# maybeLx/MVSFormerPlusPlus

Measured on NVIDIA H100. Metric: depth-maps/sec (hot path: FMT + 4-stage cascade), higher is better.
Workload: dtype f32

## Files before the change

### mvsformerplusplus_b200/csrc/attention_fa.cuh

```cuda
#pragma once

namespace fa {
using namespace gmma;
constexpr int NCONS = 256, THREADS = NCONS + 32, NKV = 3;
constexpr uint32_t TILE = 4096;
constexpr uint32_t LBO_QK = 2048, LBO_V = 640;
constexpr uint32_t V_TILE = 16 * LBO_V;
constexpr uint32_t OFF_Q = 0, OFF_K = 2 * TILE, OFF_V = OFF_K + NKV * 2 * TILE, OFF_BAR = OFF_V + NKV * V_TILE;
constexpr uint32_t SMEM = OFF_BAR + 8 + 32 * NKV;
}

__global__ void qkv_tile_kernel(const float* __restrict__ qkv, __half* __restrict__ tiled, int N, int ntiles, float qscale) {
  const int i = blockIdx.x * blockDim.x + threadIdx.x;
  const int total = ntiles * 128 * 3 * 4 * 2;
  if (i >= total) return;
  const int oct = i & 1, h = (i >> 1) & 3, which = (i >> 3) % 3, tok = i / 24;
  const size_t plane = (size_t)4 * ntiles * 2048;
  const int tile = tok >> 7, r = tok & 127;
  float v[8];
  if (tok < N) {
    const float4 a = ldg4(qkv + (size_t)tok * 192 + which * 64 + h * 16 + oct * 8);
    const float4 b = ldg4(qkv + (size_t)tok * 192 + which * 64 + h * 16 + oct * 8 + 4);
    v[0] = a.x; v[1] = a.y; v[2] = a.z; v[3] = a.w; v[4] = b.x; v[5] = b.y; v[6] = b.z; v[7] = b.w;
    if (which == 0) {
#pragma unroll
      for (int e = 0; e < 8; ++e) v[e] *= qscale;
    }
  } else {
#pragma unroll
    for (int e = 0; e < 8; ++e) v[e] = 0.f;
  }
  if (which < 2) {
    __half* ph = tiled + (size_t)(which * 2) * plane + ((size_t)h * ntiles + tile) * 2048;
    __half* pl = ph + plane;
    split_store8(ph + oct * 1024 + r * 8, pl + oct * 1024 + r * 8, v);
  } else {
    __half* pv = tiled + (size_t)4 * plane + ((size_t)h * ntiles + tile) * 5120;
    const int kc = r >> 3, e = r & 7;
#pragma unroll
    for (int d = 0; d < 8; ++d) {
      __half hi, lo;
      split_f16(v[d], hi, lo);
      pv[kc * 320 + (oct * 8 + d) * 8 + e] = lo;
      pv[kc * 320 + (16 + oct * 8 + d) * 8 + e] = hi;
    }
    if (oct == 0) {
      pv[kc * 320 + 32 * 8 + e] = __float2half_rn(1.0f);
    } else {
#pragma unroll
      for (int z = 33; z < 40; ++z) pv[kc * 320 + z * 8 + e] = __float2half_rn(0.f);
    }
  }
}

namespace fa {
using namespace gmma;
__device__ __forceinline__ void issue_scores(float (&S)[64], uint64_t q_hi, uint64_t q_lo, uint32_t kt) {
  const uint64_t k_hi = make_desc(kt, LBO_QK, 128), k_lo = make_desc(kt + TILE, LBO_QK, 128);
  mma_ss<128>(S, q_lo, k_hi, 0u);
  mma_ss<128>(S, q_hi, k_lo, 1u);
  mma_ss<128>(S, q_hi, k_hi, 1u);
  wg_commit();
}
template <bool PLO>
__device__ __forceinline__ void issue_pv(float (&O)[20], const uint32_t (&ph)[8][4], const uint32_t (&pl)[8][4], uint32_t vt) {
#pragma unroll
  for (int i = 0; i < 8; ++i) {
    mma_rs_n40(O, ph[i], make_desc(vt + 2 * i * LBO_V, LBO_V, 128), i > 0 ? 1u : 0u);
    if (PLO) mma_rs_n24(O + 8, pl[i], make_desc(vt + 2 * i * LBO_V + 256, LBO_V, 128), 1u);
  }
  wg_commit();
}
__device__ __forceinline__ void softmax_tile(float (&S)[64], float (&m)[2], float (&corr)[2], int j, int N, int q) {
  if (j * 128 + 128 > N) {
#pragma unroll
    for (int i = 0; i < 64; ++i)
      if (j * 128 + 8 * (i >> 2) + 2 * q + (i & 1) >= N) S[i] = -1e30f;
  }
  float mb[2];
#pragma unroll
  for (int h = 0; h < 2; ++h) {
    float pmax = -1e30f;
#pragma unroll
    for (int b = 0; b < 16; ++b) pmax = fmaxf(pmax, fmaxf(S[4 * b + 2 * h], S[4 * b + 2 * h + 1]));
    pmax = fmaxf(pmax, __shfl_xor_sync(0xffffffffu, pmax, 1));
    pmax = fmaxf(pmax, __shfl_xor_sync(0xffffffffu, pmax, 2));
    const float mx = fmaxf(m[h], pmax);
    corr[h] = ex2f(m[h] - mx);
    m[h] = mx;
    mb[h] = mx - 14.0f;
  }
#pragma unroll
  for (int i = 0; i < 64; ++i) S[i] = ex2f(S[i] - mb[(i >> 1) & 1]);
}
template <bool PLO>
__device__ __forceinline__ void pack_p(const float (&S)[64], uint32_t (&ph)[8][4], uint32_t (&pl)[8][4]) {
#pragma unroll
  for (int i = 0; i < 8; ++i)
#pragma unroll
    for (int r = 0; r < 4; ++r) {
      const float p0 = S[8 * i + 2 * r], p1 = S[8 * i + 2 * r + 1];
      const __half2 hh = __floats2half2_rn(p0, p1);
      ph[i][r] = *reinterpret_cast<const uint32_t*>(&hh);
      if (PLO) {
        const float2 hf = __half22float2(hh);
        pl[i][r] = pack_half2(p0 - hf.x, p1 - hf.y);
      }
    }
}
__device__ __forceinline__ void fold_tile(float (&o)[2][4], float (&l)[2], const float (&O)[20], const float (&corr)[2], int lane) {
#pragma unroll
  for (int h = 0; h < 2; ++h) {
#pragma unroll
    for (int b = 0; b < 2; ++b)
#pragma unroll
      for (int e = 0; e < 2; ++e) o[h][2 * b + e] = fmaf(o[h][2 * b + e], corr[h], O[4 * b + 2 * h + e] + O[4 * (b + 2) + 2 * h + e]);
    const float lt = __shfl_sync(0xffffffffu, O[16 + 2 * h], lane & ~3);
    l[h] = fmaf(l[h], corr[h], lt);
  }
}
}

template <bool PLO>
__global__ void __launch_bounds__(fa::THREADS, 1)
attention_fa_kernel(const __half* __restrict__ tiled, float* __restrict__ out, __half* __restrict__ out2, int N, int ntiles) {
  using namespace fa;
  extern __shared__ __align__(128) unsigned char smem[];
  const int tid = threadIdx.x, warp = tid >> 5, lane = tid & 31;
  const int head = blockIdx.y, qt = blockIdx.x;
  const size_t plane = (size_t)4 * ntiles * 2048;
  const __half* base = tiled + (size_t)head * ntiles * 2048;
  const uint32_t sb = smem_u32(smem);
  const uint32_t bar_q = sb + OFF_BAR, bar_kf = bar_q + 8, bar_ke = bar_kf + 8 * NKV, bar_vf = bar_ke + 8 * NKV,
                 bar_ve = bar_vf + 8 * NKV;
  if (tid == 0) {
    mbar_init(bar_q, 1);
    for (int i = 0; i < NKV; ++i) { mbar_init(bar_kf + 8 * i, 1); mbar_init(bar_ke + 8 * i, 2); mbar_init(bar_vf + 8 * i, 1); mbar_init(bar_ve + 8 * i, 2); }
    fence_barrier_init();
  }
  __syncthreads();

  if (warp == NCONS / 32) {
    if (lane == 0) {
      expect_tx(bar_q, 2 * TILE);
      bulk_load(sb + OFF_Q, base + 0 * plane + (size_t)qt * 2048, TILE, bar_q);
      bulk_load(sb + OFF_Q + TILE, base + 1 * plane + (size_t)qt * 2048, TILE, bar_q);
      for (int t = 0; t < ntiles; ++t) {
        const int s = t % NKV;
        const uint32_t par = (uint32_t)(((t / NKV) & 1) ^ 1);
        mbar_wait(bar_ke + 8 * s, par);
        expect_tx(bar_kf + 8 * s, 2 * TILE);
        bulk_load(sb + OFF_K + (2 * s) * TILE, base + 2 * plane + (size_t)t * 2048, TILE, bar_kf + 8 * s);
        bulk_load(sb + OFF_K + (2 * s + 1) * TILE, base + 3 * plane + (size_t)t * 2048, TILE, bar_kf + 8 * s);
        mbar_wait(bar_ve + 8 * s, par);
        expect_tx(bar_vf + 8 * s, V_TILE);
        bulk_load(sb + OFF_V + s * V_TILE, tiled + 4 * plane + ((size_t)head * ntiles + t) * (V_TILE / 2), V_TILE, bar_vf + 8 * s);
      }
    }
    return;
  }
  const int wg = warp >> 2, wq = warp & 3, q = lane & 3;
  const bool leader = (tid & 127) == 0;
  const uint64_t q_hi = make_desc(sb + OFF_Q + wg * 1024, LBO_QK, 128), q_lo = make_desc(sb + OFF_Q + TILE + wg * 1024, LBO_QK, 128);
  float o[2][4];
  float m[2] = {-1e30f, -1e30f}, l[2] = {0.f, 0.f};
#pragma unroll
  for (int h = 0; h < 2; ++h)
#pragma unroll
    for (int d = 0; d < 4; ++d) o[h][d] = 0.f;
  float S[64], O[20], corr[2];
  uint32_t ph[8][4], pl[8][4];
  mbar_wait(bar_q, 0u);
  mbar_wait(bar_kf, 0u);
  wg_fence();
  issue_scores(S, q_hi, q_lo, sb + OFF_K);
  wg_wait<0>();
  fence_regs<64>(S);
  if (leader) mbar_arrive(bar_ke);
  softmax_tile(S, m, corr, 0, N, q);
  pack_p<PLO>(S, ph, pl);
  if (ntiles > 1) {
    mbar_wait(bar_kf + 8, 0u);
    mbar_wait(bar_vf, 0u);
  }
  for (int j = 0; j + 1 < ntiles; ++j) {
    const int s = j % NKV, s1 = (j + 1) % NKV, s2 = (j + 2) % NKV;
    wg_fence();
    issue_scores(S, q_hi, q_lo, sb + OFF_K + (2 * s1) * TILE);
    issue_pv<PLO>(O, ph, pl, sb + OFF_V + s * V_TILE);
    wg_wait<1>();
    fence_regs<64>(S);
    if (leader) mbar_arrive(bar_ke + 8 * s1);
    float corr1[2];
    softmax_tile(S, m, corr1, j + 1, N, q);
    if (j + 2 < ntiles) mbar_wait(bar_kf + 8 * s2, (uint32_t)(((j + 2) / NKV) & 1));
    mbar_wait(bar_vf + 8 * s1, (uint32_t)(((j + 1) / NKV) & 1));
    wg_wait<0>();
    fence_regs<20>(O);
    if (leader) mbar_arrive(bar_ve + 8 * s);
    fold_tile(o, l, O, corr, lane);
    pack_p<PLO>(S, ph, pl);
    corr[0] = corr1[0];
    corr[1] = corr1[1];
  }
  {
    const int j = ntiles - 1, s = j % NKV;
    mbar_wait(bar_vf + 8 * s, (uint32_t)((j / NKV) & 1));
    wg_fence();
    issue_pv<PLO>(O, ph, pl, sb + OFF_V + s * V_TILE);
    wg_wait<0>();
    fence_regs<20>(O);
    fold_tile(o, l, O, corr, lane);
  }
#pragma unroll
  for (int h = 0; h < 2; ++h) {
    const int r = qt * 128 + 64 * wg + 16 * wq + (lane >> 2) + 8 * h;
    if (r >= N) continue;
    const float inv = __fdiv_rn(1.0f, l[h]);
#pragma unroll
    for (int b = 0; b < 2; ++b) {
      const int col = head * 16 + 8 * b + 2 * q;
      const float r0 = o[h][2 * b] * inv, r1 = o[h][2 * b + 1] * inv;
      if (out) *reinterpret_cast<float2*>(out + (size_t)r * 64 + col) = make_float2(r0, r1);
      if (out2) split_store2(out2 + (size_t)r * 128 + col, out2 + (size_t)r * 128 + 64 + col, r0, r1);
    }
  }
}
```

### mvsformerplusplus_b200/csrc/costreg_tr.cu

```cuda
#include <cuda_fp16.h>
#include <float.h>

#include "linear_tc.cuh"
#include "wgmma.cuh"

namespace mvsf {

constexpr int TR_PE = 0, TR_DOWN_W = 192, TR_DOWN_B = TR_DOWN_W + 64 * 256, TR_DOWN_LNW = TR_DOWN_B + 64,
              TR_DOWN_LNB = TR_DOWN_LNW + 64, TR_LAYER0 = TR_DOWN_LNB + 64;
constexpr int L_QKV = 0, L_PROJ_W = 192 * 64, L_PROJ_B = L_PROJ_W + 64 * 64, L_G1 = L_PROJ_B + 64, L_N1W = L_G1 + 64,
              L_N1B = L_N1W + 64, L_F1W = L_N1B + 64, L_F1B = L_F1W + 256 * 64, L_F2W = L_F1B + 256,
              L_F2B = L_F2W + 64 * 256, L_G2 = L_F2B + 64, L_N2W = L_G2 + 64, L_N2B = L_N2W + 64, TR_LAYER = L_N2B + 64;
constexpr int U_W = 0, U_B = 256 * 64, U_LNW = U_B + 256, U_LNB = U_LNW + 8, U_PW = U_LNB + 8, U_PB = U_PW + 8;

__global__ void pe3d_add_kernel(float* __restrict__ vol, const float* __restrict__ pos, const float* __restrict__ pe_w,
                                size_t nvox) {
  __shared__ float w[8 * 24];
  for (int i = threadIdx.x; i < 192; i += blockDim.x) w[i] = __ldg(pe_w + i);
  __syncthreads();
  size_t i = (size_t)blockIdx.x * blockDim.x + threadIdx.x;
  if (i >= nvox) return;
  const float div[4] = {1.0f, 0.1f, 0.01f, 0.001f};
  float pe[24];
#pragma unroll
  for (int a = 0; a < 3; ++a) {
    float p = __ldg(pos + a * nvox + i);
#pragma unroll
    for (int k = 0; k < 4; ++k) {
      float arg = __fmul_rn(__fmul_rn(p, 4.0f), div[k]);
      pe[a * 8 + 2 * k] = sinf(arg);
      pe[a * 8 + 2 * k + 1] = cosf(arg);
    }
  }
  float4* v = reinterpret_cast<float4*>(vol + i * 8);
  float4 v0 = v[0], v1 = v[1];
  float o[8] = {v0.x, v0.y, v0.z, v0.w, v1.x, v1.y, v1.z, v1.w};
#pragma unroll
  for (int c = 0; c < 8; ++c) {
    float s = 0.f;
#pragma unroll
    for (int k = 0; k < 24; ++k) s = fmaf(w[c * 24 + k], pe[k], s);
    o[c] += s;
  }
  v[0] = make_float4(o[0], o[1], o[2], o[3]);
  v[1] = make_float4(o[4], o[5], o[6], o[7]);
}

__global__ void patch_gather_kernel(const float* __restrict__ vol, __half* __restrict__ patches2, int D, int H, int W) {
  const int Hp = H / 4, Wp = W / 4;
  size_t total = (size_t)(D / 2) * Hp * Wp * 32;
  size_t i = (size_t)blockIdx.x * blockDim.x + threadIdx.x;
  if (i >= total) return;
  int vox = (int)(i & 31);
  size_t t = i >> 5;
  int wp = (int)(t % Wp), hp = (int)((t / Wp) % Hp), dp = (int)(t / ((size_t)Wp * Hp));
  int kw = vox & 3, kh = (vox >> 2) & 3, kd = vox >> 4;
  const float* src = vol + (((size_t)(dp * 2 + kd) * H + hp * 4 + kh) * W + wp * 4 + kw) * 8;
  float4 a = ldg4(src), b = ldg4(src + 4);
  float v[8] = {a.x, a.y, a.z, a.w, b.x, b.y, b.z, b.w};
  __half* row = patches2 + t * 512 + vox * 8;
  split_store8(row, row + 256, v);
}

__device__ __forceinline__ uint32_t pack_f16x2(float lo_elem, float hi_elem) {
  uint32_t r;
  asm("cvt.rn.f16x2.f32 %0, %1, %2;" : "=r"(r) : "f"(hi_elem), "f"(lo_elem));
  return r;
}
__device__ __forceinline__ float2 unpack_f16x2(uint32_t u) {
  __half2 h = *reinterpret_cast<__half2*>(&u);
  return __half22float2(h);
}
__device__ __forceinline__ void split_f16(float x, __half& hi, __half& lo) {
  hi = __float2half_rn(x);
  lo = __float2half_rn(x - __half2float(hi));
}
__device__ __forceinline__ float ex2f(float x) {
  float y;
  asm("ex2.approx.ftz.f32 %0, %1;" : "=f"(y) : "f"(x));
  return y;
}

#include "attention_fa.cuh"

__global__ void unpatch_ln_prob_kernel(const float* __restrict__ u, const float* __restrict__ tail,
                                       float* __restrict__ logits, int D, int H, int W) {
  const int Hp = H / 4, Wp = W / 4;
  size_t total = (size_t)D * H * W;
  size_t i = (size_t)blockIdx.x * blockDim.x + threadIdx.x;
  if (i >= total) return;
  int vox = (int)(i & 31);
  size_t t = i >> 5;
  int wp = (int)(t % Wp), hp = (int)((t / Wp) % Hp), dp = (int)(t / ((size_t)Wp * Hp));
  int kw = vox & 3, kh = (vox >> 2) & 3, kd = vox >> 4;
  float4 a = ldg4(u + i * 8), b = ldg4(u + i * 8 + 4);
  float x[8] = {a.x, a.y, a.z, a.w, b.x, b.y, b.z, b.w};
  float mean = 0.f;
#pragma unroll
  for (int c = 0; c < 8; ++c) mean += x[c];
  mean *= 0.125f;
  float var = 0.f;
#pragma unroll
  for (int c = 0; c < 8; ++c) { float dd = x[c] - mean; var = fmaf(dd, dd, var); }
  var *= 0.125f;
  const float sd = sqrtf(var + 1e-6f);
  float s = __ldg(tail + (U_PB - U_LNW));
#pragma unroll
  for (int c = 0; c < 8; ++c) {
    float y = __ldg(tail + c) * __fdiv_rn(x[c] - mean, sd) + __ldg(tail + 8 + c);
    s = fmaf(y, __ldg(tail + 16 + c), s);
  }
  logits[((size_t)(dp * 2 + kd) * H + hp * 4 + kh) * W + wp * 4 + kw] = s;
}


static int g_attention_plo = 0;

static int run_attention(const float* qkv, float* o, __half* o2, __half* tiled, int N, float scale_log2e, cudaStream_t s) {
  const int ntiles = cdiv(N, 128);
  qkv_tile_kernel<<<cdiv((long long)ntiles * 128 * 24, 256), 256, 0, s>>>(qkv, tiled, N, ntiles, scale_log2e);
  MVSF_LAUNCH_CHECK("qkv_tile");
  static DeviceOnce once;
  const int dev = current_device();
  if (once.need(dev)) {
    MVSF_CUDA_OK(cudaFuncSetAttribute(attention_fa_kernel<true>, cudaFuncAttributeMaxDynamicSharedMemorySize, (int)fa::SMEM));
    MVSF_CUDA_OK(cudaFuncSetAttribute(attention_fa_kernel<false>, cudaFuncAttributeMaxDynamicSharedMemorySize, (int)fa::SMEM));
    once.done(dev);
  }
  cudaEvent_t kt = ktimer_enabled() ? ktimer_begin("attention_tc", s) : nullptr;
  const dim3 grid(ntiles, 4);
  if (g_attention_plo)
    attention_fa_kernel<true><<<grid, fa::THREADS, fa::SMEM, s>>>(tiled, o, o2, N, ntiles);
  else
    attention_fa_kernel<false><<<grid, fa::THREADS, fa::SMEM, s>>>(tiled, o, o2, N, ntiles);
  if (kt) ktimer_end(kt, s);
  MVSF_LAUNCH_CHECK("attention_tc");
  return MVSF_OK;
}

}

using namespace mvsf;

extern "C" {

int mvsf_costreg_tr_workspace_bytes(int C, int D, int H, int W, size_t* bytes) {
  MVSF_REQUIRE(bytes && C == 8, "costreg_tr: base channel must be 8");
  MVSF_REQUIRE(D % 2 == 0 && H % 4 == 0 && W % 4 == 0 && D > 0 && H > 0 && W > 0,
               "costreg_tr: D %% 2, H %% 4, W %% 4 must be 0 (down_rate (2,4,4))");
  size_t N = (size_t)(D / 2) * (H / 4) * (W / 4);
  *bytes = (N * (256 + 64 + 64 + 64 + 64 + 64 + 192) + (N + 128) * 224) * sizeof(float);
  return MVSF_OK;
}

int mvsf_costreg_tr_forward(float* volume, const float* pos, const float* wts, const void* wts16, size_t n_wts,
                            float* logits, void* workspace, size_t workspace_bytes, int C, int D, int H, int W,
                            int layers, float softmax_scale, mvsf_stream_t stream) {
  MVSF_REQUIRE(volume && wts && wts16 && logits && workspace && layers >= 0, "costreg_tr: bad arguments");
  size_t need = 0;
  int rc = mvsf_costreg_tr_workspace_bytes(C, D, H, W, &need);
  if (rc) return rc;
  if (workspace_bytes < need) return fail(MVSF_ERR_WORKSPACE, "costreg_tr: workspace %zu < %zu bytes", workspace_bytes, need);
  MVSF_REQUIRE(((uintptr_t)workspace & 15) == 0 && ((uintptr_t)wts & 15) == 0 && ((uintptr_t)volume & 15) == 0 &&
                   ((uintptr_t)wts16 & 15) == 0 && (n_wts % 8) == 0,
               "costreg_tr: pointers must be 16-byte aligned");
  MVSF_REQUIRE(n_wts >= (size_t)TR_LAYER0 + (size_t)layers * TR_LAYER + U_PB + 1, "costreg_tr: weight blob too small");
  cudaStream_t s = (cudaStream_t)stream;
  const size_t nvox = (size_t)D * H * W;
  const int N = (int)((size_t)(D / 2) * (H / 4) * (W / 4));
  const __half* wh = reinterpret_cast<const __half*>(wts16);
  const __half* wl = wh + n_wts;
  float* big = (float*)workspace;
  __half* big2 = reinterpret_cast<__half*>(big);
  float* x = big + (size_t)N * 256;
  float* y = x + (size_t)N * 64;
  __half* x2 = reinterpret_cast<__half*>(y + (size_t)N * 64);
  __half* y2 = x2 + (size_t)N * 128;
  __half* o2 = y2 + (size_t)N * 128;
  float* qkv = reinterpret_cast<float*>(o2 + (size_t)N * 128);
  __half* split = reinterpret_cast<__half*>(qkv + (size_t)N * 192);

  if (pos) {
    pe3d_add_kernel<<<cdiv((long long)nvox, 256), 256, 0, s>>>(volume, pos, wts + TR_PE, nvox);
    MVSF_LAUNCH_CHECK("pe3d_add");
  }
  patch_gather_kernel<<<cdiv((long long)N * 32, 256), 256, 0, s>>>(volume, big2, D, H, W);
  MVSF_LAUNCH_CHECK("patch_gather");

  TcLinArgs a{};
  a.Ah = big2; a.Al = big2 + 256; a.lda = 512; a.Bh = wh + TR_DOWN_W; a.Bl = wl + TR_DOWN_W; a.ldb = 256;
  a.M = N; a.N = 64; a.K = 256; a.bias = wts + TR_DOWN_B; a.ln_w = wts + TR_DOWN_LNW; a.ln_b = wts + TR_DOWN_LNB; a.ln_eps = 1e-6f;
  a.C = x; a.ldc = 64; a.C2 = x2; a.ldc2 = 128;
  if ((rc = launch_linear_tc(a, LIN_LN, s))) return rc;

  const float scale_log2e = softmax_scale * 1.4426950408889634f;
  for (int l = 0; l < layers; ++l) {
    const size_t lo = (size_t)TR_LAYER0 + (size_t)l * TR_LAYER;
    const float* lw = wts + lo;
    TcLinArgs q{};
    q.Ah = x2; q.Al = x2 + 64; q.lda = 128; q.Bh = wh + lo + L_QKV; q.Bl = wl + lo + L_QKV; q.ldb = 64;
    q.M = N; q.N = 192; q.K = 64; q.C = qkv; q.ldc = 192;
    if ((rc = launch_linear_tc(q, LIN_BIAS, s))) return rc;
    if ((rc = run_attention(qkv, nullptr, o2, split, N, scale_log2e, s))) return rc;
    TcLinArgs p{};
    p.Ah = o2; p.Al = o2 + 64; p.lda = 128; p.Bh = wh + lo + L_PROJ_W; p.Bl = wl + lo + L_PROJ_W; p.ldb = 64;
    p.M = N; p.N = 64; p.K = 64; p.bias = lw + L_PROJ_B; p.res = x; p.ldres = 64; p.gamma = lw + L_G1;
    p.ln_w = lw + L_N1W; p.ln_b = lw + L_N1B; p.ln_eps = 1e-5f; p.C = y; p.ldc = 64; p.C2 = y2; p.ldc2 = 128;
    if ((rc = launch_linear_tc(p, LIN_RES_LN, s))) return rc;
    TcLinArgs f1{};
    f1.Ah = y2; f1.Al = y2 + 64; f1.lda = 128; f1.Bh = wh + lo + L_F1W; f1.Bl = wl + lo + L_F1W; f1.ldb = 64;
    f1.M = N; f1.N = 256; f1.K = 64; f1.bias = lw + L_F1B; f1.C2 = big2; f1.ldc2 = 512;
    if ((rc = launch_linear_tc(f1, LIN_GELU, s))) return rc;
    TcLinArgs f2{};
    f2.Ah = big2; f2.Al = big2 + 256; f2.lda = 512; f2.Bh = wh + lo + L_F2W; f2.Bl = wl + lo + L_F2W; f2.ldb = 256;
    f2.M = N; f2.N = 64; f2.K = 256; f2.bias = lw + L_F2B; f2.res = y; f2.ldres = 64; f2.gamma = lw + L_G2;
    f2.ln_w = lw + L_N2W; f2.ln_b = lw + L_N2B; f2.ln_eps = 1e-5f; f2.C = x; f2.ldc = 64; f2.C2 = x2; f2.ldc2 = 128;
    if ((rc = launch_linear_tc(f2, LIN_RES_LN, s))) return rc;
  }
  const size_t uo = (size_t)TR_LAYER0 + (size_t)layers * TR_LAYER;
  TcLinArgs u{};
  u.Ah = x2; u.Al = x2 + 64; u.lda = 128; u.Bh = wh + uo + U_W; u.Bl = wl + uo + U_W; u.ldb = 64;
  u.M = N; u.N = 256; u.K = 64; u.bias = wts + uo + U_B; u.C = big; u.ldc = 256;
  if ((rc = launch_linear_tc(u, LIN_BIAS, s))) return rc;
  unpatch_ln_prob_kernel<<<cdiv((long long)nvox, 256), 256, 0, s>>>(big, wts + uo + U_LNW, logits, D, H, W);
  MVSF_LAUNCH_CHECK("unpatch_ln_prob");
  return MVSF_OK;
}

int mvsf_attention_set_precision(int p_lo) {
  g_attention_plo = p_lo != 0;
  return MVSF_OK;
}

int mvsf_attention_forward(const float* qkv, float* out, void* workspace, size_t workspace_bytes, int N,
                           float softmax_scale, mvsf_stream_t stream) {
  MVSF_REQUIRE(qkv && out && workspace && N > 0, "attention_forward: bad arguments");
  if (workspace_bytes < (size_t)(N + 128) * 896) return fail(MVSF_ERR_WORKSPACE, "attention_forward: workspace %zu < %zu bytes", workspace_bytes, (size_t)(N + 128) * 896);
  return run_attention(qkv, out, nullptr, reinterpret_cast<__half*>(workspace), N, softmax_scale * 1.4426950408889634f, (cudaStream_t)stream);
}
}
```

Before: 43.72.

## Use three consumer warpgroups per attention CTA with register reallocation

Templates the flash-attention kernel on the number of consumer warpgroups and uses three (each owning 64 query rows) in the default non-PLO path, so each CTA amortizes K/V tile loads across 192 queries instead of 128. The Q layout is re-tiled per warpgroup with separate bulk loads, and mbarrier arrive counts scale with the warpgroup count. setmaxnreg is used to shrink the producer warpgroup's registers and grow the consumers'. Fewer CTAs reduce K/V smem traffic, but fewer blocks may underfill SMs for small N, and the padded last block clamps to reload a valid tile.

```diff
diff --git a/mvsformerplusplus_b200/csrc/attention_fa.cuh b/mvsformerplusplus_b200/csrc/attention_fa.cuh
--- a/mvsformerplusplus_b200/csrc/attention_fa.cuh
+++ b/mvsformerplusplus_b200/csrc/attention_fa.cuh
@@ -2,12 +2,13 @@
 
 namespace fa {
 using namespace gmma;
-constexpr int NCONS = 256, THREADS = NCONS + 32, NKV = 3;
+constexpr int NKV = 3;
 constexpr uint32_t TILE = 4096;
-constexpr uint32_t LBO_QK = 2048, LBO_V = 640;
+constexpr uint32_t LBO_QK = 2048, LBO_Q = 1024, LBO_V = 640;
 constexpr uint32_t V_TILE = 16 * LBO_V;
-constexpr uint32_t OFF_Q = 0, OFF_K = 2 * TILE, OFF_V = OFF_K + NKV * 2 * TILE, OFF_BAR = OFF_V + NKV * V_TILE;
-constexpr uint32_t SMEM = OFF_BAR + 8 + 32 * NKV;
+constexpr uint32_t OFF_K = 0, OFF_V = OFF_K + NKV * 2 * TILE, OFF_Q = OFF_V + NKV * V_TILE;
+constexpr int threads(int nwg) { return 128 * (nwg + 1); }
+constexpr uint32_t smem_bytes(int nwg) { return OFF_Q + nwg * TILE + 8 + 32 * NKV; }
 }
 
 __global__ void qkv_tile_kernel(const float* __restrict__ qkv, __half* __restrict__ tiled, int N, int ntiles, float qscale) {
@@ -121,30 +122,36 @@
 }
 }
 
-template <bool PLO>
-__global__ void __launch_bounds__(fa::THREADS, 1)
+template <bool PLO, int NWG>
+__global__ void __launch_bounds__(fa::threads(NWG), 1)
 attention_fa_kernel(const __half* __restrict__ tiled, float* __restrict__ out, __half* __restrict__ out2, int N, int ntiles) {
   using namespace fa;
   extern __shared__ __align__(128) unsigned char smem[];
   const int tid = threadIdx.x, warp = tid >> 5, lane = tid & 31;
-  const int head = blockIdx.y, qt = blockIdx.x;
+  const int head = blockIdx.y;
   const size_t plane = (size_t)4 * ntiles * 2048;
   const __half* base = tiled + (size_t)head * ntiles * 2048;
   const uint32_t sb = smem_u32(smem);
-  const uint32_t bar_q = sb + OFF_BAR, bar_kf = bar_q + 8, bar_ke = bar_kf + 8 * NKV, bar_vf = bar_ke + 8 * NKV,
+  const uint32_t bar_q = sb + OFF_Q + NWG * TILE, bar_kf = bar_q + 8, bar_ke = bar_kf + 8 * NKV, bar_vf = bar_ke + 8 * NKV,
                  bar_ve = bar_vf + 8 * NKV;
   if (tid == 0) {
     mbar_init(bar_q, 1);
-    for (int i = 0; i < NKV; ++i) { mbar_init(bar_kf + 8 * i, 1); mbar_init(bar_ke + 8 * i, 2); mbar_init(bar_vf + 8 * i, 1); mbar_init(bar_ve + 8 * i, 2); }
+    for (int i = 0; i < NKV; ++i) { mbar_init(bar_kf + 8 * i, 1); mbar_init(bar_ke + 8 * i, NWG); mbar_init(bar_vf + 8 * i, 1); mbar_init(bar_ve + 8 * i, NWG); }
     fence_barrier_init();
   }
   __syncthreads();
 
-  if (warp == NCONS / 32) {
-    if (lane == 0) {
-      expect_tx(bar_q, 2 * TILE);
-      bulk_load(sb + OFF_Q, base + 0 * plane + (size_t)qt * 2048, TILE, bar_q);
-      bulk_load(sb + OFF_Q + TILE, base + 1 * plane + (size_t)qt * 2048, TILE, bar_q);
+  if (warp >= 4 * NWG) {
+    if constexpr (NWG == 3) asm volatile("setmaxnreg.dec.sync.aligned.u32 32;");
+    if (warp == 4 * NWG && lane == 0) {
+      expect_tx(bar_q, NWG * TILE);
+      for (int w = 0; w < NWG; ++w) {
+        const int b = min(NWG * (int)blockIdx.x + w, 2 * ntiles - 1);
+        for (int p = 0; p < 2; ++p)
+          for (int kc = 0; kc < 2; ++kc)
+            bulk_load(sb + OFF_Q + w * TILE + p * (TILE / 2) + kc * LBO_Q,
+                      base + p * plane + (size_t)(b >> 1) * 2048 + kc * 1024 + (b & 1) * 512, LBO_Q, bar_q);
+      }
       for (int t = 0; t < ntiles; ++t) {
         const int s = t % NKV;
         const uint32_t par = (uint32_t)(((t / NKV) & 1) ^ 1);
@@ -159,9 +166,10 @@
     }
     return;
   }
+  if constexpr (NWG == 3) asm volatile("setmaxnreg.inc.sync.aligned.u32 160;");
   const int wg = warp >> 2, wq = warp & 3, q = lane & 3;
   const bool leader = (tid & 127) == 0;
-  const uint64_t q_hi = make_desc(sb + OFF_Q + wg * 1024, LBO_QK, 128), q_lo = make_desc(sb + OFF_Q + TILE + wg * 1024, LBO_QK, 128);
+  const uint64_t q_hi = make_desc(sb + OFF_Q + wg * TILE, LBO_Q, 128), q_lo = make_desc(sb + OFF_Q + wg * TILE + TILE / 2, LBO_Q, 128);
   float o[2][4];
   float m[2] = {-1e30f, -1e30f}, l[2] = {0.f, 0.f};
 #pragma unroll
@@ -214,7 +222,7 @@
   }
 #pragma unroll
   for (int h = 0; h < 2; ++h) {
-    const int r = qt * 128 + 64 * wg + 16 * wq + (lane >> 2) + 8 * h;
+    const int r = 64 * (NWG * (int)blockIdx.x + wg) + 16 * wq + (lane >> 2) + 8 * h;
     if (r >= N) continue;
     const float inv = __fdiv_rn(1.0f, l[h]);
 #pragma unroll
diff --git a/mvsformerplusplus_b200/csrc/costreg_tr.cu b/mvsformerplusplus_b200/csrc/costreg_tr.cu
--- a/mvsformerplusplus_b200/csrc/costreg_tr.cu
+++ b/mvsformerplusplus_b200/csrc/costreg_tr.cu
@@ -116,6 +116,11 @@
 
 static int g_attention_plo = 0;
 
+template <bool PLO, int NWG>
+static void launch_attention(const __half* tiled, float* o, __half* o2, int N, int ntiles, cudaStream_t s) {
+  attention_fa_kernel<PLO, NWG><<<dim3(cdiv(N, 64 * NWG), 4), fa::threads(NWG), fa::smem_bytes(NWG), s>>>(tiled, o, o2, N, ntiles);
+}
+
 static int run_attention(const float* qkv, float* o, __half* o2, __half* tiled, int N, float scale_log2e, cudaStream_t s) {
   const int ntiles = cdiv(N, 128);
   qkv_tile_kernel<<<cdiv((long long)ntiles * 128 * 24, 256), 256, 0, s>>>(qkv, tiled, N, ntiles, scale_log2e);
@@ -123,16 +128,15 @@
   static DeviceOnce once;
   const int dev = current_device();
   if (once.need(dev)) {
-    MVSF_CUDA_OK(cudaFuncSetAttribute(attention_fa_kernel<true>, cudaFuncAttributeMaxDynamicSharedMemorySize, (int)fa::SMEM));
-    MVSF_CUDA_OK(cudaFuncSetAttribute(attention_fa_kernel<false>, cudaFuncAttributeMaxDynamicSharedMemorySize, (int)fa::SMEM));
+    MVSF_CUDA_OK(cudaFuncSetAttribute(attention_fa_kernel<true, 2>, cudaFuncAttributeMaxDynamicSharedMemorySize, (int)fa::smem_bytes(2)));
+    MVSF_CUDA_OK(cudaFuncSetAttribute(attention_fa_kernel<false, 3>, cudaFuncAttributeMaxDynamicSharedMemorySize, (int)fa::smem_bytes(3)));
     once.done(dev);
   }
   cudaEvent_t kt = ktimer_enabled() ? ktimer_begin("attention_tc", s) : nullptr;
-  const dim3 grid(ntiles, 4);
   if (g_attention_plo)
-    attention_fa_kernel<true><<<grid, fa::THREADS, fa::SMEM, s>>>(tiled, o, o2, N, ntiles);
+    launch_attention<true, 2>(tiled, o, o2, N, ntiles, s);
   else
-    attention_fa_kernel<false><<<grid, fa::THREADS, fa::SMEM, s>>>(tiled, o, o2, N, ntiles);
+    launch_attention<false, 3>(tiled, o, o2, N, ntiles, s);
   if (kt) ktimer_end(kt, s);
   MVSF_LAUNCH_CHECK("attention_tc");
   return MVSF_OK;
```

Result: faster. 45.57 (median of 6 runs) (+4.2%).
